# JuliaNeuralGraphics/GaussianSplatting.jl

Measured on AMD Instinct MI355X. Metric: fwd+bwd Mpixels/s @1920x1080, 1M Gaussians SH=3, higher is better.
Workload: dtype f32

## Files before the change

gaussiansplatting.jl_amd/_lib.py:

```python
from __future__ import annotations

import ctypes as C
import os
import subprocess

_HERE = os.path.dirname(os.path.abspath(__file__))
LIB_PATH = os.environ.get("GSR_HIP_LIB", os.path.join(_HERE, "libgsr_hip.so"))
HEADER_PATH = os.path.join(os.path.dirname(_HERE), "include", "gsr.h")

GSR_OK, GSR_E_INVALID_ARG, GSR_E_OOM, GSR_E_HIP, GSR_E_STATE = 0, -1, -2, -3, -4
DEFAULT = 0
SSIM_FAST, SSIM_EXACT = 1, 2
PREPROCESS_DIRECT, PREPROCESS_AGGREGATING = 1, 2
TUNER_OFF, TUNER_ON = 1, 2
GRAD_FP32_REFERENCE, GRAD_ACCURATE = 1, 2
MODES = {"rgb": 3, "rgbd": 5, "rgbdn": 8}
FORWARD_ONLY = 1
FLAG_REFERENCE_TILE_LISTS = 2
ABI_VERSION = 6

(BUF_RADII, BUF_GRAD_MEANS2D, BUF_N_CONTRIB, BUF_FINAL_T, BUF_TILE_RANGES, BUF_VALUES_SORTED, BUF_GEOM, BUF_NORMALS,
 BUF_GRAD_ROWS, BUF_INSTANCE_AUX) = range(10)


class GsrError(RuntimeError):
    def __init__(self, code, msg):
        super().__init__(f"gsr error {code}: {msg}")
        self.code = code


class Config(C.Structure):
    _fields_ = [("width", C.c_int32), ("height", C.c_int32), ("mode", C.c_int32), ("near_plane", C.c_float),
                ("far_plane", C.c_float), ("radius_clip", C.c_int32), ("blur_eps", C.c_float), ("flags", C.c_uint32),
                ("bins_budget_bytes", C.c_uint64), ("ssim_precision", C.c_int32), ("preprocess_form", C.c_int32),
                ("form_tuner", C.c_int32), ("grad_precision", C.c_int32)]


class Inputs(C.Structure):
    _fields_ = [("n", C.c_int32), ("n_coeffs", C.c_int32), ("sh_degree", C.c_int32), ("means", C.c_void_p),
                ("shs", C.c_void_p), ("opacities", C.c_void_p), ("scales", C.c_void_p), ("rotations", C.c_void_p),
                ("background", C.c_float * 3)]


class CameraS(C.Structure):
    _fields_ = [("R", C.c_float * 9), ("t", C.c_float * 3), ("focal", C.c_float * 2), ("principal", C.c_float * 2),
                ("camera_center", C.c_float * 3), ("R_dev", C.c_void_p), ("t_dev", C.c_void_p)]


class Aux(C.Structure):
    _fields_ = [("covisibilities", C.c_void_p), ("uncertainties", C.c_void_p), ("radii", C.c_void_p),
                ("flags", C.c_uint32), ("reserved", C.c_uint32)]


class Stats(C.Structure):
    _fields_ = [("n_rendered", C.c_int64), ("n_visible", C.c_int32), ("max_tile_instances", C.c_int32),
# ... 297 lines not shown
```

gaussiansplatting.jl_amd/csrc/composite.hip:

```cpp
#include "gsr_kernels.h"
#include "gsr_dispatch.h"
#include "wave_reduce.h"
#include "tile_sort_device.h"


namespace {

struct Bg { float v[8]; };

__device__ __forceinline__ unsigned long long wave_ballot(bool p) { return __builtin_amdgcn_ballot_w64(p); }

struct SigmaX { float hxx, bdx; };
__device__ __forceinline__ SigmaX sigma_x(float ha, float b, float dx) {
    return SigmaX{__fmul_rn(ha, __fmul_rn(dx, dx)), __fmul_rn(b, dx)};
}
__device__ __forceinline__ float sigma_of(const SigmaX sx, float hc, float dy, float dy2) {
    return __fmaf_rn(sx.bdx, dy, __fmaf_rn(hc, dy2, sx.hxx));
}
__device__ __forceinline__ float alpha_of(float opacity, float G) { return fminf(0.99f, __fmul_rn(opacity, G)); }

template <int C, int N> struct LdsSplats {
    float4 q[C > 3 ? 4 : 3][N];
    __device__ __forceinline__ const float4& operator()(int plane, int j) const { return q[plane][j]; }
    __device__ __forceinline__ float4& operator()(int plane, int j) { return q[plane][j]; }
// ... 41 lines not shown
    if constexpr (C == 3 && AUX)  asm volatile(GSR_FWD_REGION(GSR_FWD_RGB GSR_FWD_UNC) : GSR_FWD_OUT_RGB, [unc] "+v"(p.unc) : GSR_FWD_IN_RGB : "scc");
    if constexpr (C == 5 && !AUX) asm volatile(GSR_FWD_REGION(GSR_FWD_RGB GSR_FWD_D) : GSR_FWD_OUT_D : GSR_FWD_IN_D : "scc");
    if constexpr (C == 5 && AUX)  asm volatile(GSR_FWD_REGION(GSR_FWD_RGB GSR_FWD_D GSR_FWD_UNC) : GSR_FWD_OUT_D, [unc] "+v"(p.unc) : GSR_FWD_IN_D : "scc");
    if constexpr (C == 8 && !AUX) asm volatile(GSR_FWD_REGION(GSR_FWD_RGB GSR_FWD_D GSR_FWD_N) : GSR_FWD_OUT_N : GSR_FWD_IN_N : "scc");
    if constexpr (C == 8 && AUX)  asm volatile(GSR_FWD_REGION(GSR_FWD_RGB GSR_FWD_D GSR_FWD_N GSR_FWD_UNC) : GSR_FWD_OUT_N, [unc] "+v"(p.unc) : GSR_FWD_IN_N : "scc");
}

template <int C, bool AUX, int N>
__device__ __forceinline__ void fwd_blend_selected(FwdPixel<C>& p, unsigned long long m, const LdsSplats<C, N>& e, int e0, float fx, float fy,
                                                   const uint32_t* __restrict__ ids, uint8_t* __restrict__ covis) {
    while (m) {
        const int jb = __builtin_ctzll(m), j = e0 + jb;
        m &= m - 1;
        float4 c2 = make_float4(0.0f, 0.0f, 0.0f, 0.0f);
        c2 = e(2, j);
        const float4 a = e(0, j), b = e(1, j);
        const float4 c3 = C > 3 ? e(C > 3 ? 3 : 0, j) : c2;
        const float dx = a.x - fx, dy = a.y - fy;
        const float sigma = sigma_of(sigma_x(a.z, a.w, dx), b.x, dy, __fmul_rn(dy, dy));
        const float alpha = alpha_of(b.y, __expf(-sigma));
        const float Tn = p.T * (1.0f - alpha);
        const unsigned long long small = wave_ballot(Tn < 1e-4f);
        const unsigned long long touch = wave_ballot(__float_as_uint(sigma) < __float_as_uint(C == 3 ? c2.z : c3.w));
        const unsigned long long okpre = touch & ~p.done;
        const unsigned long long stop = okpre & small;
        p.done |= stop;
        const unsigned long long ok = okpre ^ stop;
        float f[C];
        unpack_features<C>(b, c2, c3, f);
        const float w = alpha * p.T;
        const unsigned long long seen = AUX ? ok & wave_ballot(p.T > 0.5f) & (covis ? ~0ull : 0ull) : 0ull;
        fwd_update_under_exec<C, AUX>(p, ok, Tn, c2.y, w, f);
        if (AUX && __builtin_amdgcn_inverse_ballot_w64(seen)) covis[ids[jb]] = 1;
    }
}

template <int C, bool AUX>
__device__ __forceinline__ void fwd_pixel_store(const FwdPixel<C>& p, bool inside, int px, int py, int W, const Bg& bg,
                                                float* __restrict__ image, uint32_t* __restrict__ n_contrib,
                                                float* __restrict__ final_T, float* __restrict__ uncert) {
    if (inside) {
        const size_t pi = (size_t)px + (size_t)W * py;
        final_T[pi] = p.T;
        n_contrib[pi] = p.last;
#pragma unroll
        for (int c = 0; c < C; c++) image[(size_t)C * pi + c] = p.color[c] + p.T * bg.v[c];
        if (AUX && uncert) uncert[pi] = p.unc;
    }
}

template <int C, bool AUX>
__device__ __forceinline__ void composite_fwd_quadrant(int W, int H, int grid_x, int tile, int quad, int lane,
                                                       const uint32_t* __restrict__ tile_start, GsrStream stream,
                                                       const Bg& bg, float* __restrict__ image,
                                                       uint32_t* __restrict__ n_contrib, float* __restrict__ final_T,
                                                       const uint32_t* __restrict__ values_sorted,
                                                       uint8_t* __restrict__ covis, float* __restrict__ uncert,
                                                       LdsSplats<C, 64>& e) {
    const int tile_x = tile % grid_x, tile_y = tile / grid_x;
    const uint32_t strip_bits = 0x10000u << quad;
    const int px = tile_x * GSR_TILE + 8 * (quad & 1) + (lane & 7), py = tile_y * GSR_TILE + 8 * (quad >> 1) + (lane >> 3);
    const bool inside = px < W && py < H;
    const float fx = (float)px, fy = (float)py;
    const uint32_t start = tile_start[tile], end = tile_start[tile + 1];
    const int to_do = (int)(end - start);
    FwdPixel<C> p;
// ... 34 lines not shown
    __shared__ LdsSplats<C, 64> e;
    const int id = blockIdx.x, k = id >> 3;
    const int quad = k & 3;
    const int slot = ((k >> 2) << 3) | (id & 7);
    int tile;
    if (tile_order) {
        if (slot >= grid_x * ((H + GSR_TILE - 1) / GSR_TILE)) return;
        tile = (int)tile_order[slot];
    } else {
        if ((uint32_t)slot >= tiers.n_big + tiers.n_mid8 + tiers.n_mid4) return;
        GSR_TIER_TILE(tile, tiers, (uint32_t)slot);
        if (tiers.split_len) __builtin_amdgcn_s_setprio(3);
    }
    composite_fwd_quadrant<C, AUX>(W, H, grid_x, tile, quad, (int)threadIdx.x, tile_start, stream, bg, image,
                                   n_contrib, final_T, values_sorted, covis, uncert, e);
}

template <int C, bool AUX, bool KEEP>
__global__ __launch_bounds__(256) __attribute__((amdgpu_waves_per_eu(8))) void sort_composite_fwd_kernel(int W, int H, int grid_x,
                                                                 const uint32_t* __restrict__ tile_start,
                                                                 const uint32_t* __restrict__ tile_order,
                                                                 uint32_t* __restrict__ tile_count,
                                                                 const uint64_t* __restrict__ bins, uint32_t bin_cap,
                                                                 GsrGeom geom, GsrStream stream, Bg bg,
                                                                 float* __restrict__ image,
                                                                 uint32_t* __restrict__ n_contrib,
                                                                 float* __restrict__ final_T,
                                                                 uint32_t* __restrict__ values_sorted,
                                                                 uint32_t* __restrict__ ranges,
                                                                 uint8_t* __restrict__ covis, float* __restrict__ uncert,
                                                                 const uint32_t* __restrict__ totals,
                                                                 uint32_t cap_instances) {
    constexpr int CHUNK = 256;
    __shared__ uint32_t ids[1024];
    __shared__ LdsSplats<C, CHUNK> e;
    if (totals[GSR_TOTAL_D] > cap_instances || (totals[GSR_TOTAL_MAX_LIST] > bin_cap && bin_cap < 1024u)) return;
    const int tile = (int)tile_order[blockIdx.x];
    const int tid = threadIdx.x, lane = tid & 63, wave = tid >> 6;
    const uint32_t start = tile_start[tile], end = tile_start[tile + 1];
    const uint32_t n = end - start;
    if (tid == 0) {
        tile_count[tile] = 0u;
        ranges[2 * tile] = n ? start : 0u;
        ranges[2 * tile + 1] = n ? end : 0u;
    }
    if (n > 1024u) return;
    const int tile_x = tile % grid_x, tile_y = tile / grid_x;
    const int X0 = tile_x * GSR_TILE, Y0 = tile_y * GSR_TILE;
    const int quad = wave;
    const uint32_t strip_bits = 0x10000u << quad;
    const int px = X0 + 8 * (quad & 1) + (lane & 7), py = Y0 + 8 * (quad >> 1) + (lane >> 3);
    const bool inside = px < W && py < H;
    float fx = (float)px, fy = (float)py;
    asm volatile("" : "+v"(fx), "+v"(fy));
    FwdPixel<C> p;
    fwd_pixel_init<C>(p, inside);
    if (n > 0) {
        if (wave == (int)(blockIdx.x & 3u)) gsr_sort::wave_sort_ids_any(ids, n, lane, bins + (size_t)tile * bin_cap);
        __syncthreads();
        for (uint32_t cbase = 0; cbase < n; cbase += CHUNK) {
            const uint32_t i = cbase + (uint32_t)tid;
            if (i < n) {
                const uint32_t id = ids[i];
                const gsr_sort::InstanceVals v = gsr_sort::instance_vals<C>(id, X0, Y0, geom);
                if (KEEP) {
                    const uint32_t pos = start + i;
                    values_sorted[pos] = id;
                    stream.s0[pos] = v.v0; stream.s1[pos] = v.v1; stream.s2[pos] = v.v2;
                    if (C > 3) stream.s3[pos] = v.v3;
                }
                e(0, tid) = v.v0; e(1, tid) = v.v1;
                e(2, tid) = make_float4(v.v2.x, __uint_as_float(i + 1u), v.v2.z, v.v2.w);
                if (C > 3) e(C > 3 ? 3 : 0, tid) = v.v3;
            }
            __syncthreads();
            const int cnt = (int)min((uint32_t)CHUNK, n - cbase);
            for (int b = 0; b < cnt; b += 64) {
                if (p.done == ~0ull) break;
                const int k = b + lane;
                const bool cand = k < cnt && (__float_as_uint(e(2, k).w) & strip_bits) != 0u;
                const unsigned long long m = wave_ballot(cand);
                if (m == 0ull) continue;
                fwd_blend_selected<C, AUX, CHUNK>(p, m, e, b, fx, fy, ids + cbase + b, covis);
            }
            if (cbase + CHUNK < n) __syncthreads();
        }
    }
    fwd_pixel_store<C, AUX>(p, inside, px, py, W, bg, image, n_contrib, final_T, uncert);
}

template <int C> struct AccRow { static constexpr int N = C == 3 ? 9 : (C == 5 ? 10 : 13); static constexpr int STRIDE = N | 1; };

template <bool ACC> __device__ __forceinline__ float bwd_exp_neg(float sigma) { return ACC ? expf(-sigma) : __expf(-sigma); }
template <bool ACC> __device__ __forceinline__ float bwd_rcp(float x) { return ACC ? __fdiv_rn(1.0f, x) : __builtin_amdgcn_rcpf(x); }


template <int C, int VC>
__device__ __forceinline__ void bwd_store_row(float4* rows, const float4 a, const float4 b, float slot,
                                              const float (&r)[AccRow<VC>::N]) {
    constexpr int NA = AccRow<VC>::N;
    const float mo = -b.y, mh = -0.5f * b.y;
    float4* row = rows + (size_t)GSR_ROW_F4(C) * __float_as_uint(slot);
    row[0] = make_float4(r[0], r[1], r[2], r[3]);
    row[1] = make_float4(mh * r[4], mh * r[5], mh * r[6], VC > 3 ? r[9 < NA ? 9 : 0] : 0.0f);
    row[2] = make_float4(mo * (2.0f * a.z * r[7] + a.w * r[8]), mo * (a.w * r[7] + 2.0f * b.x * r[8]),
                         VC > 5 ? r[10 < NA ? 10 : 0] : 0.0f, VC > 5 ? r[11 < NA ? 11 : 0] : 0.0f);
    if (C > 5) row[3] = make_float4(VC > 5 ? r[12 < NA ? 12 : 0] : 0.0f, 0.0f, 0.0f, 0.0f);
}

template <int C>
__device__ __forceinline__ void bwd_zero_rows(float4* rows, const GsrStream stream, uint32_t p, uint32_t end) {
    for (; p < end; p += 64) {
        float4* row = rows + (size_t)GSR_ROW_F4(C) * __float_as_uint(stream.s2[p].y);
        const float4 z = make_float4(0.0f, 0.0f, 0.0f, 0.0f);
        row[0] = z; row[1] = z; row[2] = z;
        if (C > 5) row[3] = z;
    }
}

template <int C>
__device__ __forceinline__ uint32_t bwd_stage_entry(const GsrStream& stream, uint32_t p, int k, float4* l0, float4* l1,
// ... 161 lines not shown
bool bg_is_zero(const Bg& b) {
    for (int c = 0; c < 8; c++)
        if (b.v[c] != 0.0f) return false;
    return true;
}

Bg make_bg(const float* background, int channels) {
    Bg b;
    for (int c = 0; c < 8; c++) b.v[c] = (c < 3 && c < channels) ? background[c] : 0.0f;
    return b;
}

}

void gsr_launch_composite_fwd(hipStream_t s, int channels, GsrCam cam, GsrTiles tiles, GsrStream stream, GsrFrame frame,
                              const GsrTierLists* only_listed) {
    const uint32_t* const tile_order = only_listed ? nullptr : tiles.order;
    const GsrTierLists tiers = only_listed ? *only_listed : GsrTierLists{};
    const int n_slots = tile_order ? cam.grid_x * cam.grid_y : (int)(tiers.n_big + tiers.n_mid8 + tiers.n_mid4);
    if (n_slots <= 0) return;
    dim3 grid(32 * ((n_slots + 7) / 8)), block(64);
    Bg bg = make_bg(frame.background, channels);
    gsr::dispatch_channels(channels, [&](auto c) {
        constexpr int CH = c;
        gsr::dispatch_bool(frame.covis || frame.uncert, [&](auto a) {
            constexpr bool AUX = a;
            hipLaunchKernelGGL((composite_fwd_strip_kernel<CH, AUX>), grid, block, 0, s, cam.width, cam.height, cam.grid_x,
                               tiles.start, tile_order, stream, bg, frame.image, frame.n_contrib, frame.final_T,
                               frame.values_sorted, frame.covis, frame.uncert, tiers);
        });
    });
}

void gsr_launch_sort_composite_fwd(hipStream_t s, int channels, GsrCam cam, GsrTiles tiles, GsrKeys keys, GsrGeom geom,
                                   GsrStream stream, GsrFrame frame, uint32_t cap_instances, bool keep_backward_state) {
    dim3 grid(cam.grid_x * cam.grid_y), block(256);
    Bg bg = make_bg(frame.background, channels);
    gsr::dispatch_channels(channels, [&](auto c) {
        constexpr int CH = c;
        gsr::dispatch_bool(frame.covis || frame.uncert, [&](auto a) {
            constexpr bool AUX = a;
            gsr::dispatch_bool(keep_backward_state, [&](auto k) {
                constexpr bool KEEP = k;
                hipLaunchKernelGGL((sort_composite_fwd_kernel<CH, AUX, KEEP>), grid, block, 0, s, cam.width, cam.height,
                                   cam.grid_x, tiles.start, tiles.order, tiles.count, keys.bins, keys.cap, geom, stream, bg,
                                   frame.image, frame.n_contrib, frame.final_T, frame.values_sorted, tiles.ranges,
                                   frame.covis, frame.uncert, tiles.totals, cap_instances);
            });
        });
    });
}

void gsr_launch_composite_bwd(hipStream_t s, int channels, GsrCam cam, GsrTiles tiles, GsrStream stream, GsrFrame frame,
                              const float* vpixels, GsrInst inst, uint32_t split_len, bool color_only, bool accurate) {
    dim3 grid(cam.grid_x * cam.grid_y), block(64);
    Bg bg = make_bg(frame.background, channels);
    GsrTierLists none{};
    none.split_len = split_len;
    const bool bg0 = bg_is_zero(bg);
#define LAUNCH_K(CC, ZZ, VV, AA)                                                                                       \
    hipLaunchKernelGGL((composite_bwd_kernel<CC, ZZ, VV, AA>), grid, block, 0, s, cam.width, cam.height,               \
                       cam.grid_x, tiles.start, tiles.order, stream, bg, vpixels, frame.n_contrib, frame.final_T, inst, none)
#define LAUNCH2(CC, ZZ) do { if (accurate) LAUNCH_K(CC, false, CC, true); else LAUNCH_K(CC, ZZ, CC, false); } while (0)
#define LAUNCH3(CC, ZZ) do { if (accurate) LAUNCH_K(CC, false, 3, true); else LAUNCH_K(CC, ZZ, 3, false); } while (0)
    if (channels == 3) {
        if (bg0 && !accurate)
// ... 34 lines not shown
```

gaussiansplatting.jl_amd/csrc/gsr_api.cpp:

```cpp
#include <algorithm>
#include <atomic>
#include <cstdlib>
#include <new>

#include "gsr_kernels.h"
#include "adam_math.h"
#include "gsr_host.h"
#include "gsr_devbuf.h"
#include "gsr_profiler.h"
#include "gsr_host_wait.h"
#include "gsr_sizes.h"

using namespace gsr_host;

thread_local char gsr_host::g_err[512] = "";

namespace {

struct TunerEvents {
    hipEvent_t ev[2 * GSR_TUNER_TIMED_VIEWS] = {};
    bool create() {
        for (auto& e : ev)
            if (!e && hipEventCreate(&e) != hipSuccess) { e = nullptr; return false; }
        return true;
// ... 745 lines not shown
    gsr_launch_pergauss_bwd(s, n, in->n_coeffs, in->sh_degree, C, in->means, in->scales, in->rotations, in->shs, k,
                            geom_of(h), inst_of(h), h->vmean2d_cur, g->vmeans, g->vshs, g->vopacities,
                            g->vscales, g->vrotations, g->vR, g->vt, h->pose_part.as<float>(), g->vcolors,
                            h->cfg.grad_precision == GSR_GRAD_FP32_REFERENCE);
    sc8.close();
    HIPCHK(hipGetLastError());
    h->bwd_valid = true;
    return GSR_OK;
}

static int buffer_lookup(const gsr_handle* h, int which, const void** dev_ptr, size_t* bytes) {
    const size_t n = (size_t)h->last_n, P = (size_t)h->cfg.width * h->cfg.height, T = (size_t)h->n_tiles;
    const gsr_gaussian_bytes gb = n ? gaussian_bytes(h, h->last_n) : gsr_gaussian_bytes{};
    const gsr_instance_bytes ib = gsr_sizes_per_instance((uint64_t)h->last_D, (uint64_t)h->last_slots, h->cfg.mode);
    const DevBuf* b = nullptr;
    size_t sz = 0;
    switch (which) {
        case GSR_BUF_RADII:
            *dev_ptr = h->fwd_valid && n ? h->radii_cur : nullptr;
            *bytes = *dev_ptr ? gb.radii : 0;
            return GSR_OK;
        case GSR_BUF_GRAD_MEANS2D:
            *dev_ptr = h->bwd_valid && n ? h->vmean2d_cur : nullptr;
            *bytes = *dev_ptr ? gb.vmean2d : 0;
            return GSR_OK;
        case GSR_BUF_N_CONTRIB: b = &h->n_contrib; sz = P * 4; break;
        case GSR_BUF_FINAL_T: b = &h->final_T; sz = P * 4; break;
        case GSR_BUF_TILE_RANGES: b = &h->ranges; sz = 2 * T * 4; break;
        case GSR_BUF_VALUES_SORTED: b = &h->values_sorted; sz = h->fwd_only ? 0 : ib.values_sorted; break;
        case GSR_BUF_GEOM: b = &h->geo; sz = gb.geo; break;
        case GSR_BUF_NORMALS: b = &h->gnormal; sz = gb.gnormal; break;
        case GSR_BUF_GRAD_ROWS: b = &h->rows; sz = (size_t)h->last_slots * 16 * GSR_ROW_F4(h->cfg.mode); break;
        case GSR_BUF_INSTANCE_AUX: b = &h->s2; sz = h->fwd_only ? 0 : ib.stream; break;
        default: return fail(GSR_E_INVALID_ARG, "unknown buffer id %d", which);
    }
    if (sz > b->cap) sz = 0;
    *dev_ptr = sz ? b->p : nullptr;
    *bytes = sz;
    return GSR_OK;
}

int gsr_buffer(const gsr_handle* h, int which, const void** dev_ptr, size_t* bytes) {
    if (!h || !dev_ptr || !bytes) return fail(GSR_E_INVALID_ARG, "null argument");
    return buffer_lookup(h, which, dev_ptr, bytes);
}

int gsr_copy_buffer(const gsr_handle* h, int which, void* dst, size_t bytes, void* stream) {
    if (!h || (!dst && bytes)) return fail(GSR_E_INVALID_ARG, "null argument");
    const void* src = nullptr;
    size_t have = 0;
    int rc = buffer_lookup(h, which, &src, &have);
    if (rc) return rc;
    if (bytes > have) return fail(GSR_E_STATE, "buffer %d holds %zu bytes, %zu requested (not produced yet?)", which, have, bytes);
    if (bytes) HIPCHK(hipMemcpyAsync(dst, src, bytes, hipMemcpyDeviceToDevice, (hipStream_t)stream));
    return GSR_OK;
}

int gsr_loss_l1_ssim(gsr_handle* h, const float* image, const float* target, float lambda_dssim, float* loss_out,
                     float* vpixels, void* stream) {
    if (!h || !image || !target || !loss_out || !vpixels) return fail(GSR_E_INVALID_ARG, "null argument");
    hipStream_t s = (hipStream_t)stream;
    const int W = h->cfg.width, H = h->cfg.height, C = h->cfg.mode;
    const size_t P = (size_t)W * H;
    if (P * C > 0xFFFFFFFFull) return fail(GSR_E_INVALID_ARG, "image too large for the loss head");
    const int exact = ssim_exact_of(h);
    int rc;
    if ((rc = h->d0.ensure(3 * P * 4)) || (rc = h->d1.ensure(3 * P * 4)) || (rc = h->d2.ensure(3 * P * 4)) ||
        (rc = h->partial.ensure((exact ? gsr_loss_partial_pairs_exact : gsr_loss_partial_pairs_fast)(W, H) * 2 * 4)))
        return rc;
    const float C1 = 0.01f * 0.01f, C2 = 0.03f * 0.03f;
    StageScope sc9(h->prof, ST_LOSS_FWD, s);
    (exact ? gsr_launch_loss_fwd_exact : gsr_launch_loss_fwd_fast)(s, W, H, C, image, target, C1, C2, h->d0.as<float>(),
                                                                          h->d1.as<float>(), h->d2.as<float>(), h->partial.as<float>());
    sc9.close();
    StageScope sc10(h->prof, ST_LOSS_BWD, s);
    (exact ? gsr_launch_loss_bwd_exact : gsr_launch_loss_bwd_fast)(s, W, H, C, image, target, lambda_dssim, h->d0.as<float>(),
                                                                          h->d1.as<float>(), h->d2.as<float>(), h->partial.as<float>(),
                                                                          loss_out, vpixels);
    sc10.close();
    HIPCHK(hipGetLastError());
    h->loss_vpixels = vpixels;
    h->loss_generation = h->generation;
    return GSR_OK;
}

int gsr_update_stats(gsr_handle* h, int32_t* max_radii, float* accum_grad_means2d, float* denom, void* stream) {
// ... 103 lines not shown
```

gaussiansplatting.jl_amd/csrc/gsr_kernels.h:

```cpp
#pragma once
#include <hip/hip_runtime.h>
#include <stdint.h>

#define GSR_TILE 16
#define GSR_BATCH 256
#define GSR_SORT_LDS_CAP 8192

struct GsrCam {
    float R[9];
    float t[3];
    float focal[2];
    float principal[2];
    float center[3];
    int width, height;
    int grid_x, grid_y;
    float near_plane, far_plane;
    int radius_clip;
    float blur_eps;
    int exact_cull;
    const float* R_dev;
    const float* t_dev;
};

struct GsrGeoRec { float4 q0, q1, q2, q3; };
// ... 73 lines not shown
                              const float* vrot, const gsr::TailState& S);

void gsr_launch_update_stats(hipStream_t s, int n, const int32_t* radii, const float2* vmean2d, int width, int height,
                             int32_t* max_radii, float* accum, float* denom);

void gsr_launch_tile_scan(hipStream_t s, GsrTiles tiles, GsrGeom geom, int n_blocks, const uint32_t* bvis,
                          uint32_t* host_mirror , uint32_t seq);
void gsr_launch_tile_sort(hipStream_t s, int channels, bool main_pass, GsrTiles tiles, GsrKeys keys, uint32_t n_mid4,
                          uint32_t n_mid8, uint32_t n_big, uint32_t first4, uint32_t first8,
                          uint64_t* big_scratch , size_t slab_stride,
                          GsrGeom geom, GsrStream stream, uint32_t* values_sorted);
void gsr_launch_tile_sort_mid(hipStream_t s, int channels, GsrTiles tiles, GsrKeys keys, uint32_t grid4, uint32_t grid8,
                              GsrGeom geom, GsrStream stream, uint32_t* values_sorted, uint32_t cap_instances);

void gsr_launch_fill_background(hipStream_t s, size_t n_pixels, int channels, GsrFrame frame);
struct GsrTierLists {
    const uint32_t* lists;
    uint32_t n_tiles, n_big, n_mid8, n_mid4;
    uint32_t split_len;
};
#define GSR_TIER_TILE(tile, tiers, slot)                                                                                       \
    do {                                                                                                                       \
        uint32_t b_ = (slot);                                                                                                  \
        const uint32_t* list_ = (tiers).lists;                                                               \
        if (b_ >= (tiers).n_big) { b_ -= (tiers).n_big; list_ = (tiers).lists + (tiers).n_tiles;             \
            if (b_ >= (tiers).n_mid8) { b_ -= (tiers).n_mid8; list_ = (tiers).lists + 2 * (size_t)(tiers).n_tiles; } }   \
        (tile) = (int)list_[b_];                                                                                               \
    } while (0)
void gsr_launch_composite_fwd(hipStream_t s, int channels, GsrCam cam, GsrTiles tiles, GsrStream stream, GsrFrame frame,
                              const GsrTierLists* only_listed );
void gsr_launch_sort_composite_fwd(hipStream_t s, int channels, GsrCam cam, GsrTiles tiles, GsrKeys keys, GsrGeom geom,
                                   GsrStream stream, GsrFrame frame, uint32_t cap_instances,
                                   bool keep_backward_state );
void gsr_launch_composite_bwd(hipStream_t s, int channels, GsrCam cam, GsrTiles tiles, GsrStream stream, GsrFrame frame,
                              const float* vpixels, GsrInst inst,
                              uint32_t split_len ,
                              bool color_only ,
                              bool accurate );
void gsr_launch_composite_bwd_listed(hipStream_t s, int channels, GsrCam cam, GsrTiles tiles, GsrTierLists tiers,
                                     GsrStream stream, GsrFrame frame, const float* vpixels, GsrInst inst,
                                     float* long_state );

#define GSR_ADAM_MAX_GROUPS 8
void gsr_launch_prologue_fwd(hipStream_t s, int n, int k_rest, int scale_dims, const float* sh_color,
                             const float* sh_remainder, const float* opacities, const float* scales, float* shs,
                             float* opacities_act, float* scales_act);
void gsr_launch_prologue_bwd(hipStream_t s, int n, int k_rest, int scale_dims, const float* opacities_act,
                             const float* scales_act, const float* vshs, const float* vopacities_act,
                             const float* vscales_act, float* v_sh_color, float* v_sh_remainder, float* v_opacities,
                             float* v_scales);
void gsr_launch_adam(hipStream_t s, int n_groups, float* const* theta, const float* const* grad, float* const* mu,
                     float* const* nu, const long long* count, const float* lr_t, float beta1, float beta2, float eps);

void gsr_launch_trainer_tail(hipStream_t s, int n, int k_rest, int scale_dims, const float* const* grads,
                             float* const* theta, float* const* mu, float* const* nu, const float* lr_t, float beta1,
                             float beta2, float eps, float* shs, float* opac_act, float* scales_act);
size_t gsr_findall_scratch_bytes(long long n);
void gsr_launch_findall(hipStream_t s, long long n, const uint8_t* mask, uint32_t* indices, uint32_t* count_dev,
                        uint32_t* scratch);
void gsr_launch_gather_rows(hipStream_t s, int n_groups, const void* const* src, void* const* dst, const int* row_words,
                            const uint32_t* idx, long long count);
void gsr_launch_triad(hipStream_t s, size_t n4, float* a, const float* b, const float* c, float q);

#define GSR_COMPOSE_MAX_GROUPS 24
void gsr_launch_grad_mean(hipStream_t s, long long n, const float* accum, const float* denom, float* out);
void gsr_launch_densify_mask(hipStream_t s, int kind, long long n, long long n_grad, const float* grad, const float* scales,
// ... 100 lines not shown
```

gaussiansplatting.jl_amd/csrc/tile_mask.h:

```cpp
#pragma once
#include <hip/hip_runtime.h>
#include <stdint.h>

__device__ __forceinline__ uint32_t instance_row_mask(const float4 g0, const float4 g1, uint32_t X, int X0, int Y0) {
    const float mx = g0.x, my = g0.y, a = g0.z, b = g0.w, c = g1.x;
    const float ha = 0.5f * a, hc = 0.5f * c;
    const float l_hi = mx - (float)X0, l_lo = mx - (float)(X0 + 7);
    const float r_hi = mx - (float)(X0 + 8), r_lo = mx - (float)(X0 + 15);
    const float dy0 = my - (float)Y0;
    const float xm = fmaxf(fabsf(l_hi), fabsf(r_lo)), ym = fmaxf(fabsf(dy0), fabsf(dy0 - 15.0f));
    const float M = ha * (xm * xm) + fabsf(b) * (xm * ym) + hc * (ym * ym);
    const float ts = __uint_as_float(X - 1u) + 2e-3f + 4e-6f * M;
    const float nboa = -b * __builtin_amdgcn_rcpf(a);
    uint32_t ml = 0, mr = 0;
#pragma unroll
    for (int r = 15; r >= 0; r--) {
        const float dy = dy0 - (float)r;
        const float v = nboa * dy, bdy = b * dy;
        const float k = __fmaf_rn(dy, hc * dy, -ts);
        const float xl = __builtin_amdgcn_fmed3f(v, l_lo, l_hi), xr = __builtin_amdgcn_fmed3f(v, r_lo, r_hi);
        const float sl = __fmaf_rn(xl, __fmaf_rn(ha, xl, bdy), k), sr = __fmaf_rn(xr, __fmaf_rn(ha, xr, bdy), k);
        ml = __builtin_amdgcn_alignbit(ml, __float_as_uint(sl), 31);
        mr = __builtin_amdgcn_alignbit(mr, __float_as_uint(sr), 31);
    }
    uint32_t m = (ml | mr) | ((ml & 0xFFu) ? 1u << 16 : 0u) | ((mr & 0xFFu) ? 1u << 17 : 0u) |
                 ((ml & 0xFF00u) ? 1u << 18 : 0u) | ((mr & 0xFF00u) ? 1u << 19 : 0u);
    if (!(a > 0.0f)) m = 0xFFFFFu;
    if (X == 0u) m = 0u;
    return m;
}


__device__ __forceinline__ uint32_t blend_threshold_bits(float o) {
    const float amin = 1.0f / 255.0f;
    auto pass = [&](uint32_t b) { return fminf(0.99f, __fmul_rn(o, (float)exp(-(double)__uint_as_float(b)))) >= amin; };
    if (!pass(0u)) return 0u;
    const float tau = fmaxf(logf(255.0f * o), 0.0f);
    const float w = 4e-7f * fmaxf(tau, 1.0f);
    uint32_t lo = __float_as_uint(fmaxf(tau - w, 0.0f)), hi = __float_as_uint(tau + w);
    if (!pass(lo)) lo = 0u;
    for (int k = 0; k < 24 && pass(hi); k++) { lo = hi; hi = __float_as_uint(__uint_as_float(hi) + w * (float)(2 << k)); }
    if (pass(hi)) return hi + 1u;
    while (hi - lo > 1u) {
        const uint32_t mid = lo + ((hi - lo) >> 1);
        if (pass(mid)) lo = mid; else hi = mid;
    }
    return lo + 1u;
}

__device__ __forceinline__ float footprint_tau(float opacity) { return __logf(255.0f * opacity) + 2e-3f; }

__device__ __forceinline__ bool tile_may_touch(float mx, float my, float a, float b, float c, float tau, int X0,
                                               int Y0) {
    if (!(tau >= 0.0f)) return false;
    if (!(a > 0.0f) || !(c > 0.0f)) return true;
    const float x_lo = mx - (float)(X0 + 15), x_hi = mx - (float)X0;
    const float y_lo = my - (float)(Y0 + 15), y_hi = my - (float)Y0;
    if (x_lo <= 0.0f && x_hi >= 0.0f && y_lo <= 0.0f && y_hi >= 0.0f) return true;
    const float inv_a = 1.0f / a, inv_c = 1.0f / c;
    float best = 3.0e38f;
#pragma unroll
    for (int e = 0; e < 2; e++) {
// ... 10 lines not shown
```

gaussiansplatting.jl_amd/csrc/tile_sort_device.h:

```cpp
#pragma once
#include "gsr_kernels.h"
#include "tile_mask.h"

namespace gsr_sort {

struct InstanceVals { float4 v0, v1, v2, v3; };
struct InstanceRaw { GsrGeoRec rec; uint32_t bpre; float4 normal; };
template <int CH>
__device__ __forceinline__ InstanceRaw instance_load(uint32_t id, const GsrGeom& geom) {
    InstanceRaw r;
    r.rec = geom.rec[id];
    r.bpre = geom.bpre[id >> 8];
    r.normal = make_float4(0.0f, 0.0f, 0.0f, 0.0f);
    if (CH > 5) r.normal = geom.normal[id];
    return r;
}
template <int CH>
__device__ __forceinline__ InstanceVals instance_vals_of(const InstanceRaw& r, int X0, int Y0) {
    InstanceVals o;
    const GsrGeoRec& rec = r.rec;
    o.v0 = make_float4(rec.q0.x, rec.q0.y, 0.5f * rec.q0.z, rec.q0.w);
    o.v1 = make_float4(0.5f * rec.q1.x, rec.q1.y, rec.q1.z, rec.q1.w);
    const uint32_t lo = __float_as_uint(rec.q3.x), hi = __float_as_uint(rec.q3.y);
    const uint32_t x0 = lo & 0xFFFFu, y0 = lo >> 16, x1 = hi & 0xFFFFu, y1 = hi >> 16;
    const uint32_t k = ((uint32_t)(Y0 / GSR_TILE) - y0) * (x1 - x0) + ((uint32_t)(X0 / GSR_TILE) - x0);
    const uint32_t dense = (x1 - x0) * (y1 - y0) <= GSR_DENSE_RECT;
    const uint32_t rank = dense ? (uint32_t)__popc(__float_as_uint(rec.q3.w) & ((1u << (k & 31u)) - 1u)) : k;
    const uint32_t slot = r.bpre + __float_as_uint(rec.q2.w) + rank;
    const uint32_t mask_bits = instance_row_mask(rec.q0, rec.q1, __float_as_uint(rec.q3.z), X0, Y0);
    const float X = rec.q3.z;
    const float z = CH == 3 ? X : rec.q2.z;
    o.v2 = make_float4(rec.q2.x, __uint_as_float(slot), z, __uint_as_float(mask_bits));
    o.v3 = make_float4(r.normal.x, r.normal.y, r.normal.z, X);
    return o;
}
template <int CH>
__device__ __forceinline__ InstanceVals instance_vals(uint32_t id, int X0, int Y0, const GsrGeom& geom) {
    return instance_vals_of<CH>(instance_load<CH>(id, geom), X0, Y0);
}

template <int CH>
__device__ __forceinline__ void emit_instance(uint64_t k, uint32_t pos, int X0, int Y0, const GsrGeom& geom,
                                              const GsrStream& stream, uint32_t* __restrict__ values_sorted) {
    const uint32_t id = (uint32_t)k;
    values_sorted[pos] = id;
    const InstanceVals v = instance_vals<CH>(id, X0, Y0, geom);
    stream.s0[pos] = v.v0;
    stream.s1[pos] = v.v1;
    stream.s2[pos] = v.v2;
    if (CH > 3) stream.s3[pos] = v.v3;
}

__device__ __forceinline__ uint64_t shfl_xor_u64(uint64_t v, int s) {
    const uint32_t lo = (uint32_t)__shfl_xor((int)(uint32_t)v, s), hi = (uint32_t)__shfl_xor((int)(uint32_t)(v >> 32), s);
    return ((uint64_t)hi << 32) | lo;
}
template <int KPT>
__device__ __forceinline__ void wave_bitonic_sort(uint64_t (&v)[KPT], uint32_t m, int lane) {
    for (uint32_t k = 2; k <= m; k <<= 1) {
        const bool up = ((uint32_t)(lane * KPT) & k) == 0u;
        for (uint32_t j = k >> 1; j >= (uint32_t)KPT; j >>= 1) {
            const int s = (int)(j / KPT);
// ... 106 lines not shown
```

gaussiansplatting.jl_amd/rasterizer.py:

```python
from __future__ import annotations

import ctypes as C
from typing import Optional

import numpy as np
import torch

from . import _lib as L
from .camera import Camera


def n_color_features(mode: str) -> int:
    if mode not in L.MODES:
        raise ValueError(f"Invalid render mode: `{mode}`.")
    return L.MODES[mode]


def _chk(t: torch.Tensor, name: str, shape=None):
    if not t.is_cuda:
        raise ValueError(f"{name} must be a HIP device tensor (no CPU path)")
    if t.dtype != torch.float32:
        raise ValueError(f"{name} must be float32")
    if not t.is_contiguous():
        raise ValueError(f"{name} must be contiguous")
# ... 158 lines not shown
        out = torch.empty(shape, dtype=dtype, device=self.device)
        with torch.cuda.device(self.device):
            L.check(self._lib.gsr_copy_buffer(self._h, which, out.data_ptr(), n * itemsize, L.stream()))
        return out

    @property
    def radii(self):
        return self.gstate.radii

    @property
    def grad_means_2d(self):
        return self.gstate.grad_means_2d

    @property
    def n_contrib(self):
        return self._buffer(L.BUF_N_CONTRIB, torch.int32, (self.height, self.width))

    @property
    def accum_alpha(self):
        return self._buffer(L.BUF_FINAL_T, torch.float32, (self.height, self.width))

    @property
    def ranges(self):
        return self._buffer(L.BUF_TILE_RANGES, torch.int32, (self.grid[0] * self.grid[1], 2))

    @property
    def values_sorted(self):
        return self._buffer(L.BUF_VALUES_SORTED, torch.int32, (int(self.stats.n_rendered),))

    @property
    def instance_masks(self):
        d = int(self.stats.n_rendered)
        return self._buffer(L.BUF_INSTANCE_AUX, torch.int32, (d, 4))[:, 3]

    def geometry(self):
        n = self._n
        g = self._buffer(L.BUF_GEOM, torch.float32, (n, 16))
        gi = g.view(torch.int32)
        lo, hi = gi[:, 12], gi[:, 13]
        rect = torch.stack([lo & 0xFFFF, lo >> 16, hi & 0xFFFF, hi >> 16], 1)
        out = dict(means2d=g[:, 0:2], conics=g[:, 2:5], opacities=g[:, 5], rgbs=g[:, 6:9], clamped_bits=gi[:, 9],
                   depths=g[:, 10], rect=rect)
        if self.channels > 5:
            out["normals"] = self._buffer(L.BUF_NORMALS, torch.float32, (n, 4))[:, :3]
        return out

    def __call__(self, means_3d, opacities, scales, rotations, sh_color, sh_remainder, R_w2c=None, t_w2c=None, *,
                 camera: Camera, sh_degree: int, background=(0.0, 0.0, 0.0), covisibilities=None,
                 uncertainties=None):
        shs, opacities_act, scales_act = _Prologue.apply(sh_color, sh_remainder, opacities, scales)
        return rasterize(means_3d, shs, opacities_act, scales_act, rotations, R_w2c, t_w2c,
                         rast=self, camera=camera, sh_degree=sh_degree, background=background,
                         covisibilities=covisibilities, uncertainties=uncertainties)

    def _inputs(self, means_3d, shs, opacities, scales, rotations, sh_degree, background):
        n = means_3d.shape[0]
        _chk(means_3d, "means_3d", (n, 3)); _chk(scales, "scales", (n, 3)); _chk(rotations, "rotations", (n, 4))
        _chk(shs, "shs"); _chk(opacities, "opacities")
        if shs.dim() != 3 or shs.shape[0] != n or shs.shape[2] != 3:
            raise ValueError(f"shs has shape {tuple(shs.shape)}, expected (N,K,3)")
        if opacities.numel() != n:
            raise ValueError("opacities must have N elements")
        inp = L.Inputs(n, int(shs.shape[1]), int(sh_degree), means_3d.data_ptr(), shs.data_ptr(),
                       opacities.data_ptr(), scales.data_ptr(), rotations.data_ptr(),
                       (C.c_float * 3)(*[float(b) for b in background]))
        return inp
# ... 210 lines not shown
```

include/gsr.h:

```cpp
#ifndef GSR_H
#define GSR_H

#include <stddef.h>
#include <stdint.h>

#ifdef __cplusplus
extern "C" {
#endif

#define GSR_API __attribute__((visibility("default")))

enum {
    GSR_OK = 0,
    GSR_E_INVALID_ARG = -1,
    GSR_E_OOM = -2,
    GSR_E_HIP = -3,
    GSR_E_STATE = -4
};

enum { GSR_MODE_RGB = 3, GSR_MODE_RGBD = 5, GSR_MODE_RGBDN = 8 };

typedef struct gsr_config {
    int32_t width, height;
    int32_t mode;
// ... 87 lines not shown
} gsr_grads;
#define GSR_GRADS_COLOR_COTANGENT 0x1u

typedef struct gsr_handle gsr_handle;

GSR_API int gsr_create(const gsr_config* cfg, gsr_handle** out);
GSR_API int gsr_destroy(gsr_handle* h);
GSR_API int gsr_release_scene_buffers(gsr_handle* h);
GSR_API int64_t gsr_memory_usage(const gsr_handle* h);
GSR_API int gsr_debug_check_guards(gsr_handle* h);
GSR_API int gsr_reserve(gsr_handle* h, int64_t n_gaussians, int64_t n_instances);
GSR_API int gsr_drop_forward(gsr_handle* h);
GSR_API uint32_t gsr_bins_capacity_after(int64_t n_rendered, int32_t max_tile_instances, int32_t width, int32_t height,
                                         uint64_t bins_budget_bytes, uint32_t current_capacity);

GSR_API int gsr_forward(gsr_handle* h, const gsr_inputs* in, const gsr_camera* cam, float* image_out,
                        const gsr_aux* aux, void* stream, gsr_stats* stats);

GSR_API int gsr_backward(gsr_handle* h, const gsr_inputs* in, const gsr_camera* cam, const float* vpixels,
                         const gsr_grads* grads, void* stream);

GSR_API int gsr_host_wait_policy(int spin_us, int yield_us, int sleep_us);

enum {
    GSR_BUF_RADII = 0,
    GSR_BUF_GRAD_MEANS2D = 1,
    GSR_BUF_N_CONTRIB = 2,
    GSR_BUF_FINAL_T = 3,
    GSR_BUF_TILE_RANGES = 4,
    GSR_BUF_VALUES_SORTED = 5,
    GSR_BUF_GEOM = 6,
    GSR_BUF_NORMALS = 7,
    GSR_BUF_GRAD_ROWS = 8,
    GSR_BUF_INSTANCE_AUX = 9
};
GSR_API int gsr_buffer(const gsr_handle* h, int which, const void** dev_ptr, size_t* bytes);
GSR_API int gsr_copy_buffer(const gsr_handle* h, int which, void* dst, size_t bytes, void* stream);

GSR_API int gsr_update_stats(gsr_handle* h, int32_t* max_radii, float* accum_grad_means2d, float* denom, void* stream);

GSR_API int gsr_ssim_forward(int W, int H, int CH, int B, const float* img, const float* ref, float C1, float C2,
                             int train, float* ssim_map, float* dm_dmu1, float* dm_dsigma1_sq, float* dm_dsigma12,
                             void* stream);
GSR_API int gsr_ssim_backward(int W, int H, int CH, int B, const float* img, const float* ref, const float* dL_dmap,
                              const float* dm_dmu1, const float* dm_dsigma1_sq, const float* dm_dsigma12,
                              float* dL_dimg, void* stream);

GSR_API int gsr_ssim_precision(int exact);
GSR_API int gsr_get_ssim_precision(void);

GSR_API int gsr_preprocess_form(int form);
GSR_API int gsr_get_preprocess_form(void);

GSR_API int gsr_loss_l1_ssim(gsr_handle* h, const float* image, const float* target, float lambda_dssim,
                             float* loss_out, float* vpixels, void* stream);

GSR_API int gsr_prologue_forward(int32_t n, int32_t k_rest, int32_t scale_dims, const float* sh_color,
                                 const float* sh_remainder, const float* opacities, const float* scales, float* shs,
                                 float* opacities_act, float* scales_act, void* stream);
GSR_API int gsr_prologue_backward(int32_t n, int32_t k_rest, int32_t scale_dims, const float* opacities_act,
                                  const float* scales_act, const float* vshs, const float* vopacities_act,
                                  const float* vscales_act, float* v_sh_color, float* v_sh_remainder,
                                  float* v_opacities, float* v_scales, void* stream);

#define GSR_ADAM_MAX_GROUPS 8
typedef struct gsr_adam_group {
    float* theta;
// ... 198 lines not shown
```

Baseline: 1588.

## Cull splats per 4x4 pixel block with per-lane LDS visit lists in RGB forward

```diff
diff --git a/gaussiansplatting.jl_amd/_lib.py b/gaussiansplatting.jl_amd/_lib.py
--- a/gaussiansplatting.jl_amd/_lib.py
+++ b/gaussiansplatting.jl_amd/_lib.py
@@ -20,7 +20,7 @@
 ABI_VERSION = 6
 
 (BUF_RADII, BUF_GRAD_MEANS2D, BUF_N_CONTRIB, BUF_FINAL_T, BUF_TILE_RANGES, BUF_VALUES_SORTED, BUF_GEOM, BUF_NORMALS,
- BUF_GRAD_ROWS, BUF_INSTANCE_AUX) = range(10)
+ BUF_GRAD_ROWS, BUF_INSTANCE_AUX, BUF_BLOCK_MASKS) = range(11)
 
 
 class GsrError(RuntimeError):
diff --git a/gaussiansplatting.jl_amd/csrc/composite.hip b/gaussiansplatting.jl_amd/csrc/composite.hip
--- a/gaussiansplatting.jl_amd/csrc/composite.hip
+++ b/gaussiansplatting.jl_amd/csrc/composite.hip
@@ -97,6 +97,65 @@
         const unsigned long long seen = AUX ? ok & wave_ballot(p.T > 0.5f) & (covis ? ~0ull : 0ull) : 0ull;
         fwd_update_under_exec<C, AUX>(p, ok, Tn, c2.y, w, f);
         if (AUX && __builtin_amdgcn_inverse_ballot_w64(seen)) covis[ids[jb]] = 1;
+    }
+}
+
+struct FwdBlockLists {
+    uint16_t off[4][64 + 2][4];
+};
+__device__ __forceinline__ int fwd_build_block_lists(uint16_t (*wl)[4], uint32_t bits, uint32_t entry_off, uint32_t bit0, int lane,
+                                                     uint32_t sentinel_off) {
+    const unsigned long long m0 = wave_ballot((bits & bit0) != 0u), m1 = wave_ballot((bits & (bit0 << 1)) != 0u);
+    const unsigned long long m2 = wave_ballot((bits & (bit0 << 4)) != 0u), m3 = wave_ballot((bits & (bit0 << 5)) != 0u);
+    if ((m0 | m1 | m2 | m3) == 0ull) return 0;
+    __builtin_amdgcn_wave_barrier();
+    const uint32_t s2 = sentinel_off | sentinel_off << 16;
+    *reinterpret_cast<uint2*>(wl[lane]) = make_uint2(s2, s2);
+    auto rank = [](unsigned long long m) {
+        return __builtin_amdgcn_mbcnt_hi((uint32_t)(m >> 32), __builtin_amdgcn_mbcnt_lo((uint32_t)m, 0u));
+    };
+    if (bits & bit0) wl[rank(m0)][0] = (uint16_t)entry_off;
+    if (bits & (bit0 << 1)) wl[rank(m1)][1] = (uint16_t)entry_off;
+    if (bits & (bit0 << 4)) wl[rank(m2)][2] = (uint16_t)entry_off;
+    if (bits & (bit0 << 5)) wl[rank(m3)][3] = (uint16_t)entry_off;
+    __builtin_amdgcn_fence(__ATOMIC_RELEASE, "wavefront");
+    __builtin_amdgcn_wave_barrier();
+    return max(max(__popcll(m0), __popcll(m1)), max(__popcll(m2), __popcll(m3)));
+}
+
+template <int C, bool AUX, int N>
+__device__ __forceinline__ void fwd_blend_block_lists(FwdPixel<C>& p, int trip, const LdsSplats<C, N>& e, const uint16_t* lp, float fx,
+                                                      float fy, const uint32_t* __restrict__ ids, uint8_t* __restrict__ covis) {
+    static_assert(C == 3, "the block walk is the :rgb kernel's (the threshold travels in plane 2)");
+    auto visit = [&](uint32_t off) {
+        const char* const q = reinterpret_cast<const char*>(&e) + off;
+        float4 c2 = make_float4(0.0f, 0.0f, 0.0f, 0.0f);
+        c2 = *reinterpret_cast<const float4*>(q + 2 * sizeof(float4) * N);
+        const float4 a = *reinterpret_cast<const float4*>(q), b = *reinterpret_cast<const float4*>(q + sizeof(float4) * N);
+        const float dx = a.x - fx, dy = a.y - fy;
+        const float sigma = sigma_of(sigma_x(a.z, a.w, dx), b.x, dy, __fmul_rn(dy, dy));
+        const float alpha = alpha_of(b.y, __expf(-sigma));
+        const float Tn = p.T * (1.0f - alpha);
+        const unsigned long long small = wave_ballot(Tn < 1e-4f);
+        const unsigned long long touch = wave_ballot(__float_as_uint(sigma) < __float_as_uint(c2.z));
+        const unsigned long long okpre = touch & ~p.done;
+        const unsigned long long stop = okpre & small;
+        p.done |= stop;
+        const unsigned long long ok = okpre ^ stop;
+        float f[C];
+        unpack_features<C>(b, c2, c2, f);
+        const float w = alpha * p.T;
+        const unsigned long long seen = AUX ? ok & wave_ballot(p.T > 0.5f) & (covis ? ~0ull : 0ull) : 0ull;
+        fwd_update_under_exec<C, AUX>(p, ok, Tn, c2.y, w, f);
+        if (AUX && __builtin_amdgcn_inverse_ballot_w64(seen)) covis[ids[off >> 4]] = 1;
+    };
+    uint32_t o0 = lp[0], o1 = lp[4];
+    for (int t = 0; t < trip; t += 2) {
+        lp += 8;
+        visit(o0);
+        o0 = lp[0];
+        visit(o1);
+        o1 = lp[4];
     }
 }
 
@@ -197,8 +256,10 @@
                                                                  const uint32_t* __restrict__ totals,
                                                                  uint32_t cap_instances) {
     constexpr int CHUNK = 256;
+    constexpr bool LISTS = C == 3;
+    constexpr int NE = LISTS ? CHUNK + 1 : CHUNK;
     __shared__ uint32_t ids[1024];
-    __shared__ LdsSplats<C, CHUNK> e;
+    __shared__ LdsSplats<C, NE> e;
     if (totals[GSR_TOTAL_D] > cap_instances || (totals[GSR_TOTAL_MAX_LIST] > bin_cap && bin_cap < 1024u)) return;
     const int tile = (int)tile_order[blockIdx.x];
     const int tid = threadIdx.x, lane = tid & 63, wave = tid >> 6;
@@ -214,7 +275,10 @@
     const int X0 = tile_x * GSR_TILE, Y0 = tile_y * GSR_TILE;
     const int quad = wave;
     const uint32_t strip_bits = 0x10000u << quad;
-    const int px = X0 + 8 * (quad & 1) + (lane & 7), py = Y0 + 8 * (quad >> 1) + (lane >> 3);
+    const int blk = lane >> 4;
+    auto pixel_x = [&](int l, int qd) { return X0 + 8 * (qd & 1) + (LISTS ? 4 * ((l >> 4) & 1) + (l & 3) : l & 7); };
+    auto pixel_y = [&](int l, int qd) { return Y0 + 8 * (qd >> 1) + (LISTS ? 4 * (l >> 5) + ((l >> 2) & 3) : l >> 3); };
+    const int px = pixel_x(lane, quad), py = pixel_y(lane, quad);
     const bool inside = px < W && py < H;
     float fx = (float)px, fy = (float)py;
     asm volatile("" : "+v"(fx), "+v"(fy));
@@ -222,6 +286,7 @@
     fwd_pixel_init<C>(p, inside);
     if (n > 0) {
         if (wave == (int)(blockIdx.x & 3u)) gsr_sort::wave_sort_ids_any(ids, n, lane, bins + (size_t)tile * bin_cap);
+        if (LISTS && tid < 3) e(tid, NE - 1) = make_float4(0.0f, 0.0f, 0.0f, 0.0f);
         __syncthreads();
         for (uint32_t cbase = 0; cbase < n; cbase += CHUNK) {
             const uint32_t i = cbase + (uint32_t)tid;
@@ -235,23 +300,54 @@
                     if (C > 3) stream.s3[pos] = v.v3;
                 }
                 e(0, tid) = v.v0; e(1, tid) = v.v1;
-                e(2, tid) = make_float4(v.v2.x, __uint_as_float(i + 1u), v.v2.z, v.v2.w);
+                e(2, tid) = make_float4(v.v2.x, __uint_as_float(i + 1u), v.v2.z, LISTS ? __uint_as_float(v.blocks) : v.v2.w);
                 if (C > 3) e(C > 3 ? 3 : 0, tid) = v.v3;
             }
             __syncthreads();
             const int cnt = (int)min((uint32_t)CHUNK, n - cbase);
-            for (int b = 0; b < cnt; b += 64) {
-                if (p.done == ~0ull) break;
-                const int k = b + lane;
-                const bool cand = k < cnt && (__float_as_uint(e(2, k).w) & strip_bits) != 0u;
-                const unsigned long long m = wave_ballot(cand);
-                if (m == 0ull) continue;
-                fwd_blend_selected<C, AUX, CHUNK>(p, m, e, b, fx, fy, ids + cbase + b, covis);
+            if constexpr (LISTS) {
+                __shared__ FwdBlockLists lists;
+                const uint32_t bit0 = 1u << (8 * (quad >> 1) + 2 * (quad & 1));
+                for (int b = 0; b < cnt; b += 64) {
+                    if (p.done == ~0ull) break;
+                    const int k = b + lane;
+                    const uint32_t bits = k < cnt ? __float_as_uint(e(2, k).w) : 0u;
+                    const int trip = fwd_build_block_lists(lists.off[wave], bits, 16u * (uint32_t)k, bit0, lane, 16u * CHUNK);
+                    if (trip == 0) continue;
+                    fwd_blend_block_lists<C, AUX, NE>(p, trip, e, &lists.off[wave][0][blk], fx, fy, ids + cbase, covis);
+                }
+            } else {
+                for (int b = 0; b < cnt; b += 64) {
+                    if (p.done == ~0ull) break;
+                    const int k = b + lane;
+                    const bool cand = k < cnt && (__float_as_uint(e(2, k).w) & strip_bits) != 0u;
+                    const unsigned long long m = wave_ballot(cand);
+                    if (m == 0ull) continue;
+                    fwd_blend_selected<C, AUX, NE>(p, m, e, b, fx, fy, ids + cbase + b, covis);
+                }
             }
             if (cbase + CHUNK < n) __syncthreads();
         }
     }
-    fwd_pixel_store<C, AUX>(p, inside, px, py, W, bg, image, n_contrib, final_T, uncert);
+    int tid_s = tid;
+    asm volatile("" : "+v"(tid_s));
+    const int quad_s = __builtin_amdgcn_readfirstlane(tid_s >> 6);
+    const int sx = pixel_x(tid_s & 63, quad_s), sy = pixel_y(tid_s & 63, quad_s);
+    fwd_pixel_store<C, AUX>(p, sx < W && sy < H, sx, sy, W, bg, image, n_contrib, final_T, uncert);
+}
+
+__global__ __launch_bounds__(256) void block_masks_kernel(int grid_x, const uint32_t* __restrict__ ranges,
+                                                          const uint32_t* __restrict__ values_sorted, GsrGeom geom,
+                                                          uint32_t* __restrict__ out, uint32_t count) {
+    const int tile = blockIdx.x;
+    const uint32_t start = ranges[2 * tile], end = min(ranges[2 * tile + 1], count);
+    const int X0 = (tile % grid_x) * GSR_TILE, Y0 = (tile / grid_x) * GSR_TILE;
+    for (uint32_t p = start + threadIdx.x; p < end; p += 256) {
+        const GsrGeoRec rec = geom.rec[values_sorted[p]];
+        uint32_t blocks;
+        instance_footprint_masks(rec.q0, rec.q1, __float_as_uint(rec.q3.z), X0, Y0, blocks);
+        out[p] = blocks;
+    }
 }
 
 template <int C> struct AccRow { static constexpr int N = C == 3 ? 9 : (C == 5 ? 10 : 13); static constexpr int STRIDE = N | 1; };
@@ -479,6 +575,13 @@
     });
 }
 
+void gsr_launch_block_masks(hipStream_t s, GsrTiles tiles, GsrGeom geom, const uint32_t* values_sorted, uint32_t* out,
+                            uint32_t count) {
+    if (tiles.n_tiles <= 0 || count == 0) return;
+    hipLaunchKernelGGL(block_masks_kernel, dim3(tiles.n_tiles), dim3(256), 0, s, tiles.grid_x, tiles.ranges, values_sorted, geom,
+                       out, count);
+}
+
 void gsr_launch_sort_composite_fwd(hipStream_t s, int channels, GsrCam cam, GsrTiles tiles, GsrKeys keys, GsrGeom geom,
                                    GsrStream stream, GsrFrame frame, uint32_t cap_instances, bool keep_backward_state) {
     dim3 grid(cam.grid_x * cam.grid_y), block(256);
diff --git a/gaussiansplatting.jl_amd/csrc/gsr_api.cpp b/gaussiansplatting.jl_amd/csrc/gsr_api.cpp
--- a/gaussiansplatting.jl_amd/csrc/gsr_api.cpp
+++ b/gaussiansplatting.jl_amd/csrc/gsr_api.cpp
@@ -801,6 +801,10 @@
         case GSR_BUF_NORMALS: b = &h->gnormal; sz = gb.gnormal; break;
         case GSR_BUF_GRAD_ROWS: b = &h->rows; sz = (size_t)h->last_slots * 16 * GSR_ROW_F4(h->cfg.mode); break;
         case GSR_BUF_INSTANCE_AUX: b = &h->s2; sz = h->fwd_only ? 0 : ib.stream; break;
+        case GSR_BUF_BLOCK_MASKS:
+            *dev_ptr = nullptr;
+            *bytes = h->fwd_valid && !h->fwd_only && ib.values_sorted <= h->values_sorted.cap ? ib.values_sorted : 0;
+            return GSR_OK;
         default: return fail(GSR_E_INVALID_ARG, "unknown buffer id %d", which);
     }
     if (sz > b->cap) sz = 0;
@@ -821,6 +825,12 @@
     int rc = buffer_lookup(h, which, &src, &have);
     if (rc) return rc;
     if (bytes > have) return fail(GSR_E_STATE, "buffer %d holds %zu bytes, %zu requested (not produced yet?)", which, have, bytes);
+    if (which == GSR_BUF_BLOCK_MASKS) {
+        gsr_launch_block_masks((hipStream_t)stream, tiles_of(h), geom_of(h), h->values_sorted.as<uint32_t>(), (uint32_t*)dst,
+                               (uint32_t)(bytes / 4));
+        HIPCHK(hipGetLastError());
+        return GSR_OK;
+    }
     if (bytes) HIPCHK(hipMemcpyAsync(dst, src, bytes, hipMemcpyDeviceToDevice, (hipStream_t)stream));
     return GSR_OK;
 }
diff --git a/gaussiansplatting.jl_amd/csrc/gsr_kernels.h b/gaussiansplatting.jl_amd/csrc/gsr_kernels.h
--- a/gaussiansplatting.jl_amd/csrc/gsr_kernels.h
+++ b/gaussiansplatting.jl_amd/csrc/gsr_kernels.h
@@ -129,6 +129,8 @@
 void gsr_launch_sort_composite_fwd(hipStream_t s, int channels, GsrCam cam, GsrTiles tiles, GsrKeys keys, GsrGeom geom,
                                    GsrStream stream, GsrFrame frame, uint32_t cap_instances,
                                    bool keep_backward_state );
+void gsr_launch_block_masks(hipStream_t s, GsrTiles tiles, GsrGeom geom, const uint32_t* values_sorted, uint32_t* out,
+                            uint32_t count);
 void gsr_launch_composite_bwd(hipStream_t s, int channels, GsrCam cam, GsrTiles tiles, GsrStream stream, GsrFrame frame,
                               const float* vpixels, GsrInst inst,
                               uint32_t split_len ,
diff --git a/gaussiansplatting.jl_amd/csrc/tile_mask.h b/gaussiansplatting.jl_amd/csrc/tile_mask.h
--- a/gaussiansplatting.jl_amd/csrc/tile_mask.h
+++ b/gaussiansplatting.jl_amd/csrc/tile_mask.h
@@ -2,32 +2,53 @@
 #include <hip/hip_runtime.h>
 #include <stdint.h>
 
-__device__ __forceinline__ uint32_t instance_row_mask(const float4 g0, const float4 g1, uint32_t X, int X0, int Y0) {
+__device__ __forceinline__ uint32_t instance_footprint_masks(const float4 g0, const float4 g1, uint32_t X, int X0, int Y0,
+                                                             uint32_t& blocks) {
     const float mx = g0.x, my = g0.y, a = g0.z, b = g0.w, c = g1.x;
     const float ha = 0.5f * a, hc = 0.5f * c;
-    const float l_hi = mx - (float)X0, l_lo = mx - (float)(X0 + 7);
-    const float r_hi = mx - (float)(X0 + 8), r_lo = mx - (float)(X0 + 15);
+    float fX0 = (float)X0;
+    asm volatile("" : "+v"(fX0));
+    float q_hi[4], q_lo[4];
+#pragma unroll
+    for (int q = 0; q < 4; q++) { q_hi[q] = mx - (fX0 + (float)(4 * q)); q_lo[q] = mx - (fX0 + (float)(4 * q + 3)); }
     const float dy0 = my - (float)Y0;
-    const float xm = fmaxf(fabsf(l_hi), fabsf(r_lo)), ym = fmaxf(fabsf(dy0), fabsf(dy0 - 15.0f));
+    const float xm = fmaxf(fabsf(q_hi[0]), fabsf(q_lo[3])), ym = fmaxf(fabsf(dy0), fabsf(dy0 - 15.0f));
     const float M = ha * (xm * xm) + fabsf(b) * (xm * ym) + hc * (ym * ym);
     const float ts = __uint_as_float(X - 1u) + 2e-3f + 4e-6f * M;
     const float nboa = -b * __builtin_amdgcn_rcpf(a);
-    uint32_t ml = 0, mr = 0;
-#pragma unroll
-    for (int r = 15; r >= 0; r--) {
-        const float dy = dy0 - (float)r;
+    uint32_t mq[4] = {0u, 0u, 0u, 0u};
+    float fr = 15.0f;
+#pragma unroll 1
+    for (int r = 0; r < 16; r++) {
+        const float dy = dy0 - fr;
+        fr -= 1.0f;
         const float v = nboa * dy, bdy = b * dy;
         const float k = __fmaf_rn(dy, hc * dy, -ts);
-        const float xl = __builtin_amdgcn_fmed3f(v, l_lo, l_hi), xr = __builtin_amdgcn_fmed3f(v, r_lo, r_hi);
-        const float sl = __fmaf_rn(xl, __fmaf_rn(ha, xl, bdy), k), sr = __fmaf_rn(xr, __fmaf_rn(ha, xr, bdy), k);
-        ml = __builtin_amdgcn_alignbit(ml, __float_as_uint(sl), 31);
-        mr = __builtin_amdgcn_alignbit(mr, __float_as_uint(sr), 31);
+#pragma unroll
+        for (int q = 0; q < 4; q++) {
+            const float x = __builtin_amdgcn_fmed3f(v, q_lo[q], q_hi[q]);
+            const float s = __fmaf_rn(x, __fmaf_rn(ha, x, bdy), k);
+            mq[q] = __builtin_amdgcn_alignbit(mq[q], __float_as_uint(s), 31);
+        }
     }
+    const uint32_t ml = mq[0] | mq[1], mr = mq[2] | mq[3];
     uint32_t m = (ml | mr) | ((ml & 0xFFu) ? 1u << 16 : 0u) | ((mr & 0xFFu) ? 1u << 17 : 0u) |
                  ((ml & 0xFF00u) ? 1u << 18 : 0u) | ((mr & 0xFF00u) ? 1u << 19 : 0u);
-    if (!(a > 0.0f)) m = 0xFFFFFu;
-    if (X == 0u) m = 0u;
+    uint32_t bl = 0u;
+#pragma unroll
+    for (int q = 0; q < 4; q++) {
+        uint32_t t = mq[q] | (mq[q] >> 1);
+        t |= t >> 2;
+        bl |= (t & 0x1111u) << q;
+    }
+    if (!(a > 0.0f)) { m = 0xFFFFFu; bl = 0xFFFFu; }
+    if (X == 0u) { m = 0u; bl = 0u; }
+    blocks = bl;
     return m;
+}
+__device__ __forceinline__ uint32_t instance_row_mask(const float4 g0, const float4 g1, uint32_t X, int X0, int Y0) {
+    uint32_t blocks;
+    return instance_footprint_masks(g0, g1, X, X0, Y0, blocks);
 }
 
 
diff --git a/gaussiansplatting.jl_amd/csrc/tile_sort_device.h b/gaussiansplatting.jl_amd/csrc/tile_sort_device.h
--- a/gaussiansplatting.jl_amd/csrc/tile_sort_device.h
+++ b/gaussiansplatting.jl_amd/csrc/tile_sort_device.h
@@ -4,7 +4,7 @@
 
 namespace gsr_sort {
 
-struct InstanceVals { float4 v0, v1, v2, v3; };
+struct InstanceVals { float4 v0, v1, v2, v3; uint32_t blocks; };
 struct InstanceRaw { GsrGeoRec rec; uint32_t bpre; float4 normal; };
 template <int CH>
 __device__ __forceinline__ InstanceRaw instance_load(uint32_t id, const GsrGeom& geom) {
@@ -27,7 +27,7 @@
     const uint32_t dense = (x1 - x0) * (y1 - y0) <= GSR_DENSE_RECT;
     const uint32_t rank = dense ? (uint32_t)__popc(__float_as_uint(rec.q3.w) & ((1u << (k & 31u)) - 1u)) : k;
     const uint32_t slot = r.bpre + __float_as_uint(rec.q2.w) + rank;
-    const uint32_t mask_bits = instance_row_mask(rec.q0, rec.q1, __float_as_uint(rec.q3.z), X0, Y0);
+    const uint32_t mask_bits = instance_footprint_masks(rec.q0, rec.q1, __float_as_uint(rec.q3.z), X0, Y0, o.blocks);
     const float X = rec.q3.z;
     const float z = CH == 3 ? X : rec.q2.z;
     o.v2 = make_float4(rec.q2.x, __uint_as_float(slot), z, __uint_as_float(mask_bits));
diff --git a/gaussiansplatting.jl_amd/rasterizer.py b/gaussiansplatting.jl_amd/rasterizer.py
--- a/gaussiansplatting.jl_amd/rasterizer.py
+++ b/gaussiansplatting.jl_amd/rasterizer.py
@@ -214,6 +214,18 @@
     def instance_masks(self):
         d = int(self.stats.n_rendered)
         return self._buffer(L.BUF_INSTANCE_AUX, torch.int32, (d, 4))[:, 3]
+
+    @property
+    def block_masks(self):
+        d = int(self.stats.n_rendered)
+        p, sz = C.c_void_p(), C.c_size_t()
+        L.check(self._lib.gsr_buffer(self._h, L.BUF_BLOCK_MASKS, C.byref(p), C.byref(sz)))
+        if sz.value < d * 4:
+            raise RuntimeError("buffer not produced yet")
+        out = torch.empty((d,), dtype=torch.int32, device=self.device)
+        with torch.cuda.device(self.device):
+            L.check(self._lib.gsr_copy_buffer(self._h, L.BUF_BLOCK_MASKS, out.data_ptr(), d * 4, L.stream()))
+        return out
 
     def geometry(self):
         n = self._n
diff --git a/include/gsr.h b/include/gsr.h
--- a/include/gsr.h
+++ b/include/gsr.h
@@ -143,7 +143,8 @@
     GSR_BUF_GEOM = 6,
     GSR_BUF_NORMALS = 7,
     GSR_BUF_GRAD_ROWS = 8,
-    GSR_BUF_INSTANCE_AUX = 9
+    GSR_BUF_INSTANCE_AUX = 9,
+    GSR_BUF_BLOCK_MASKS = 10
 };
 GSR_API int gsr_buffer(const gsr_handle* h, int which, const void** dev_ptr, size_t* bytes);
 GSR_API int gsr_copy_buffer(const gsr_handle* h, int which, void* dst, size_t bytes, void* stream);
```

Result: no change. 1602 (median of 6 runs) (+0.9%).
